# m4drat/wtf

Hardware: AMD Instinct MI355X
Metric: execs/sec + emulated instr/s per node (tlv_server, HEVD) at 1/2/4/8 GPUs (higher is better)
Workload: dtype u64

## Files before the change

wtf_amd/csrc/engine_fast.h:

```cpp
#pragma once
#include "engine_ops.h"

namespace wtfgpu_dev {

enum : u32 {
  FO_GENERIC = 0,
  FO_NOP,
  FO_MOV,
  FO_ALU,
  FO_LEA,
  FO_INCDEC,
  FO_JCC,
  FO_JMP,
  FO_CALL,
  FO_RET,
  FO_MOVX,
  FO_SHIFT,
  FO_CMOV,
  FO_SETCC,
  FO_BT,
  FO_UNARY,
  FO_VLD,
  FO_VST,
  FO_VMOV,
  FO_VZU,
};
enum : u32 {
  FF_AREG = 1,
  FF_BREG = 2,
  FF_EA = 4,
  FF_PUSH = 8,
  FF_POP = 16,
  FF_MR_A = 32,
  FF_MR_B = 64,
  FF_MW = 128,
  FF_WRA = 256,
  FF_FLAGS = 512,
};

constexpr u32 NOREG = 16;
constexpr u32 FR_HB = 32;

struct FOp {
  u32 w0;
  u32 fl;
  u32 w2;
  u32 pad;
  u64 disp, imm;
};

__device__ __forceinline__ u32 fo_op(const FOp &f) { return f.w0 & 0xff; }
__device__ __forceinline__ u32 fo_sub(const FOp &f) { return (f.w0 >> 8) & 0xf; }
__device__ __forceinline__ u32 fo_sz(const FOp &f) { return (f.w0 >> 12) & 0xf; }
__device__ __forceinline__ u32 fo_szb(const FOp &f) { return (f.w0 >> 16) & 0xf; }
__device__ __forceinline__ u32 fo_len(const FOp &f) { return (f.w0 >> 20) & 0x3f; }
__device__ __forceinline__ u32 fo_scale(const FOp &f) { return (f.w0 >> 26) & 3; }
__device__ __forceinline__ u32 fo_riprel(const FOp &f) { return (f.w0 >> 28) & 1; }
__device__ __forceinline__ u32 fo_seg(const FOp &f) { return (f.w0 >> 29) & 3; }
__device__ __forceinline__ u32 fo_ra(const FOp &f) { return f.w2 & 0xff; }
__device__ __forceinline__ u32 fo_rb(const FOp &f) { return (f.w2 >> 8) & 0xff; }
__device__ __forceinline__ u32 fo_base(const FOp &f) { return (f.w2 >> 16) & 0xff; }
__device__ __forceinline__ u32 fo_index(const FOp &f) { return (f.w2 >> 24) & 0xff; }

__device__ __forceinline__ u32 loc_regno(const UOp &u, u32 loc) {
  switch (loc) {
    case L_GREG: return u.reg;
    case L_RM: return u.is_mem ? NOREG : u.rm;
    case L_RAX: return 0;
    case L_OPREG: return u.opreg;
    default: return NOREG;
  }
}

__device__ __forceinline__ void digest_sse(const UOp &u, u32 &op, u32 &sub, u32 &ra, u32 &rb, u32 &sz) {
  const u32 x = u.opreg, c = u.sub, pp = u.bsz;
  const bool vex = x & 1;
  if (vex_map(x) != 1 || (x & 0x30000)) return;
  const u32 vvvv = vex ? (x >> 4) & 15 : 0;
  sz = vex && ((x >> 1) & 1) ? 4 : 2;
  sub = vex ? 2 : 0;
  if (vex && c == 0x77) {
    if (sz == 2) op = FO_VZU;
    return;
  }
  const bool load = ((c == 0x6f) && (pp == 1 || pp == 2)) || ((c == 0x10 || c == 0x28) && pp <= 1);
  const bool store = ((c == 0x7f) && (pp == 1 || pp == 2)) || ((c == 0x11 || c == 0x29) && pp <= 1);
  const bool aligned = c == 0x28 || c == 0x29 || (pp == 1 && (c == 0x6f || c == 0x7f));
  if ((load || store) && vvvv == 0) {
    if (aligned) sub |= 1;
    if (!u.is_mem) op = FO_VMOV, ra = load ? u.reg : u.rm, rb = load ? u.rm : u.reg;
    else op = load ? FO_VLD : FO_VST, ra = u.reg;
    return;
  }
  if (((c == 0xef && pp == 1) || (c == 0x57 && pp <= 1)) && !u.is_mem && (vex ? vvvv : u.reg) == u.rm)
    op = FO_VMOV, sub |= 4, ra = u.reg, rb = u.rm;
}

__device__ __forceinline__ void digest(const UOp &u, FOp &f) {
  u32 op = FO_GENERIC, fl = 0, sub = u.sub;
  const u32 ra = loc_regno(u, u.asrc), rb = loc_regno(u, u.bsrc);
  const bool amem = u.asrc == L_RM && u.is_mem;
  const bool bmem = u.bsrc == L_RM && u.is_mem;
  const bool areg = ra != NOREG, breg = rb != NOREG, bimm = u.bsrc == L_IMM;
  const bool hba = !u.rex && u.asz == 1 && areg && ra >= 4 && ra < 8;
  const bool hbb = !u.rex && u.bsz == 1 && breg && rb >= 4 && rb < 8;
  const bool hb = (hba || hbb) &&
                  !(u.op == O_ALU || u.op == O_TEST || u.op == O_MOV || u.op == O_MOVZX || u.op == O_MOVSX ||
                    u.op == O_INCDEC || u.op == O_NOT || u.op == O_NEG || u.op == O_SETCC || u.op == O_SHIFT);
  u64 imm = u.imm;
  u32 ra_ = ra, rb_ = rb, sz_ = u.asz;
  if (u.op == O_SSE && u.supported && !u.seg && !u.p67) {
    digest_sse(u, op, sub, ra_, rb_, sz_);
  } else if (u.supported && !u.p67 && !u.rep && !hb) {
    switch (u.op) {
      case O_NOP: op = FO_NOP; break;
      case O_MOV:
// ... 313 lines not shown
```

wtf_amd/csrc/engine_run.h:

```cpp
#pragma once
#include <hip/hip_runtime.h>

#include "engine_fast.h"

using namespace wtfgpu_dev;

namespace {

__device__ __forceinline__ u64 wave_sum(u64 v) {
#pragma unroll
  for (int off = 32; off > 0; off >>= 1) v += __shfl_xor(v, off, 64);
  return v;
}
__device__ __forceinline__ u64 readlane64(u64 v, int l) {
  const u32 lo = __builtin_amdgcn_readlane((u32)v, l);
  const u32 hi = __builtin_amdgcn_readlane((u32)(v >> 32), l);
  return ((u64)hi << 32) | lo;
}
__device__ __forceinline__ u64 m_eq32(u32 a, u32 b) { return __builtin_amdgcn_uicmp(a, b, 32); }
__device__ __forceinline__ u64 m_ne32(u32 a, u32 b) { return __builtin_amdgcn_uicmp(a, b, 33); }
__device__ __forceinline__ u64 m_eq64(u64 a, u64 b) { return __builtin_amdgcn_uicmpl(a, b, 32); }
__device__ __forceinline__ u64 m_ne64(u64 a, u64 b) { return __builtin_amdgcn_uicmpl(a, b, 33); }
__device__ __forceinline__ u64 m_lt64(u64 a, u64 b) { return __builtin_amdgcn_uicmpl(a, b, 36); }
__device__ __forceinline__ u64 m_ge64(u64 a, u64 b) { return __builtin_amdgcn_uicmpl(a, b, 35); }
// ... 143 lines not shown

__device__ __noinline__ u32 cover_edge(const Dev &P, u64 e, bool mine, u32 lane, u32 gen, u32 cnt) {
  if (!mine) return cnt;
  if (P.extra_keys && set_has(P.extra_keys, P.extra_mask, e)) return cnt;
  return log_value(P, e, true, lane, gen, cnt);
}

__device__ __forceinline__ u32 log_value(const Dev &P, u64 rip, bool mine, u32 lane, u32 gen, u32 cnt) {
  if (!mine) return cnt;
  const u32 H = P.H;
  const u64 base = (u64)lane * H;
  u32 h = (u32)mix64(rip) & (H - 1);
  for (u32 probe = 0; probe < H; probe++) {
    const u64 idx = base + h;
    if (P.cov_gen[idx] != gen) {
      if (cnt >= H - H / 4) {
        P.cov_overflow[lane] = 1;
        return cnt;
      }
      P.cov_rip[idx] = rip;
      P.cov_gen[idx] = gen;
      return cnt + 1;
    }
    if (P.cov_rip[idx] == rip) return cnt;
    h = (h + 1) & (H - 1);
  }
  return cnt;
}

__device__ __forceinline__ void fetch_bytes(u64 pageptr, u32 off, u32 n, u64 &lo, u64 &hi) {
  const u64 a = (pageptr + off) & ~7ull;
  const u32 sh = (u32)((pageptr + off) & 7);
  const u64 pend = pageptr + WTFGPU_PAGE_SIZE;
  const u64 w0 = rfl64(*(const u64 *)a);
  const u64 w1 = (a + 8 < pend) ? rfl64(*(const u64 *)(a + 8)) : 0;
  const u64 w2 = (a + 16 < pend) ? rfl64(*(const u64 *)(a + 16)) : 0;
  if (sh == 0) {
    lo = w0;
    hi = w1;
  } else {
    lo = (w0 >> (8 * sh)) | (w1 << (64 - 8 * sh));
    hi = (w1 >> (8 * sh)) | (w2 << (64 - 8 * sh));
  }
  if (n < 16) {
    if (n <= 8) {
      hi = 0;
      lo = n == 8 ? lo : (lo & ((1ull << (8 * n)) - 1));
    } else {
      hi &= (1ull << (8 * (n - 8))) - 1;
    }
  }
}

constexpr u32 UC_N = 312;
constexpr u32 UC_U = 4;
constexpr u32 UC_BP = 1, UC_COVERED = 2, UC_CROSS = 4, UC_BADLEN = 8, UC_UNSUP = 16;
struct UCHead {
  u64 key;
  u64 logged;
  u32 flags, pad;
  FOp f;
};
struct UCEntry {
  union {
    UCHead h;
    struct {
      u64 key;
      u64 logged;
      u32 flags, pad;
      FOp f;
    };
  };
  u64 rip;
};
struct UCUop {
  u64 key;
  UOp u;
};
struct GPayload {
  u32 flags, pad;
  FOp f;
  UOp u;
};
constexpr u32 GP_HEAD = (sizeof(u32) * 2 + sizeof(FOp)) / 4;
static_assert(sizeof(UOp) % 4 == 0 && sizeof(FOp) % 4 == 0, "copied as dwords");
static_assert(sizeof(UCEntry) == 64, "LDS entry size");
constexpr u32 UC_QUEUES = 2;
constexpr u64 UC_IMAGE_BYTES = (u64)UC_N * sizeof(UCEntry);

constexpr u32 UC_WAYS = 2;
static_assert(UC_N % UC_WAYS == 0, "whole sets");
__device__ __forceinline__ bool cacheable_key(u64 lptr, u64 pool_lo, u64 pool_span) {
  return !m_ge64(lptr - pool_lo, pool_span);
}
__device__ __forceinline__ u32 uc_slot(u64 key) {
  const u32 h = ((u32)key ^ (u32)(key >> 17)) * 0x9E3779B1u;
  return __umulhi(h, UC_N / UC_WAYS) * UC_WAYS;
}
__device__ __forceinline__ u32 uu_slot(u64 key) { return (u32)((key ^ (key >> 12) * 0x9E3779B1u) & (UC_U - 1)); }

template <typename T>
__device__ __forceinline__ void lds_uniform_read(const T *src, T &dst) {
  const u32 *s = (const u32 *)src;
  u32 *d = (u32 *)&dst;
#pragma unroll
  for (u32 i = 0; i < sizeof(T) / 4; i++) d[i] = rfl32(s[i]);
}

__device__ __forceinline__ void uc_head_read(const UCEntry *e, UCHead &h) {
  h.key = rfl64(e->key);
  h.flags = rfl32(e->flags);
  h.f.w0 = rfl32(e->f.w0);
  h.f.fl = rfl32(e->f.fl);
  h.f.w2 = rfl32(e->f.w2);
  h.f.disp = rfl64(e->f.disp);
  h.f.imm = rfl64(e->f.imm);
}

__device__ __forceinline__ bool bp_lookup(const Dev &P, u64 rip) {
  u32 s;
  return P.bp_keys && hash_find(P.bp_keys, P.bp_mask, rip, s);
}

__device__ __forceinline__ bool lane_phys_write(const Dev &P, Lane &L, u64 gpa, const u8 *src, u64 len) {
  while (len) {
    const u64 off = gpa & 0xfff;
    u64 n = 4096 - off;
    if (n > len) n = len;
    bool priv;
    const u8 *pg = phys_page(P, L.lane, L.ovn, L.bloom, gpa >> 12, priv);
    u8 *dst = (u8 *)pg;
    if (!priv) {
      dst = ov_alloc(P, L.lane, L.ovn);
      if (!dst) return false;
      cow_copy(P, L.lane, L.ovn, gpa >> 12, pg, dst);
      L.ovn++;
      L.bloom |= bloom_bit(gpa >> 12);
    }
    for (u64 i = 0; i < n; i++) dst[off + i] = src[i];
    src += n;
    gpa += n;
    len -= n;
  }
  return true;
}

__device__ __forceinline__ bool lane_phys_write64(const Dev &P, Lane &L, u64 gpa, u64 v) {
  bool priv;
  const u8 *pg = phys_page(P, L.lane, L.ovn, L.bloom, gpa >> 12, priv);
  u8 *dst = (u8 *)pg;
  if (!priv) {
    dst = ov_alloc(P, L.lane, L.ovn);
    if (!dst) return false;
    cow_copy(P, L.lane, L.ovn, gpa >> 12, pg, dst);
    L.ovn++;
    L.bloom |= bloom_bit(gpa >> 12);
  }
  *(u64 *)(dst + (gpa & 0xfff)) = v;
  return true;
}

__device__ __forceinline__ bool has_error_code(u32 vec) {
  return vec == 8 || (vec >= 10 && vec <= 14) || vec == 17 || vec == 21 || vec == 29 || vec == 30;
}
__device__ __forceinline__ bool sup_xlate(const Dev &P, Lane &L, u64 va, int acc, u64 &gpa) {
  u64 td, gpfn;
  if (!walk(P, L, va, acc, td, gpfn)) return false;
  gpa = (gpfn << 12) | (va & 0xfff);
  return true;
}
// ... 53 lines not shown
    L.flush = 0;
    ok = true;
  } while (0);
  if (!ok) {
    L.cpl = cpl0;
    L.status = st0;
    L.exvec = vec;
    L.exerr = err;
    L.exaddr = cr2;
    L.nodeliver = 1;
  }
  return ok;
}

constexpr u32 GUC_WORDS = 48;
constexpr u32 GUC_PAYLOAD = sizeof(GPayload) / 4;
static_assert(GUC_PAYLOAD <= 3 * 14, "global uop cache entry: 3 lines of 14 payload dwords");
__device__ __forceinline__ u32 guc_slot(const Dev &P, u64 key) {
  return (u32)(mix64(key) & P.guc_mask);
}
__device__ __forceinline__ u32 guc_payload_index(u32 lid) {
  return (lid < GUC_WORDS && (lid & 15) < 14) ? (lid >> 4) * 14 + (lid & 15) : ~0u;
}

__device__ __forceinline__ u32 covered_flag(const Dev &P, u64 rip, u32 off) {
  if (P.code_keys) {
    u32 s;
    if (hash_find(P.code_keys, P.code_mask, rip >> 12, s)) {
      const u32 cs = rfl32(P.code_slot[s]);
      if (rfl32(P.cov_map[(u64)cs * WTFGPU_PAGE_SIZE + off])) return UC_COVERED;
    }
  }
  return 0;
}

__device__ __forceinline__ u32 covered_flag_lane(const Dev &P, u64 rip, u32 off) {
  if (!P.code_keys) return 0;
  u32 h = (u32)mix64(rip >> 12) & P.code_mask;
  for (u32 i = 0; i <= P.code_mask; i++) {
    const u64 k = P.code_keys[h];
    if (k == (rip >> 12)) return P.cov_map[(u64)P.code_slot[h] * WTFGPU_PAGE_SIZE + off] ? UC_COVERED : 0;
    if (k == EMPTY_KEY) return 0;
    h = (h + 1) & P.code_mask;
  }
  return 0;
}

__device__ __forceinline__ FOp generic_fop(const UOp &d) {
  FOp f{};
  f.w0 = (d.len & 0x3f) << 20;
  return f;
}

__device__ __forceinline__ bool uc_fill_shared(const Dev &P, UCEntry *e, UCUop *us, u64 key, u32 off, u64 rip,
                                               u32 lid) {
  if (!P.guc) return false;
  const u32 pj = guc_payload_index(lid);
  u32 *head = e ? (u32 *)&e->flags : nullptr, *uop = us ? (u32 *)&us->u : nullptr;
  u32 *gw = P.guc + (u64)guc_slot(P, key) * GUC_WORDS;
  const u32 w = lid < GUC_WORDS ? gw[lid] : 0;
  const bool tag = lid < GUC_WORDS && (lid & 15) >= 14;
  const bool bad = tag && w != ((lid & 1) ? (u32)(key >> 32) : (u32)key);
  if (__ballot(bad) != 0) return false;
  if (pj < GP_HEAD) {
    if (head) head[pj] = w;
  } else if (pj < GUC_PAYLOAD) {
    if (uop) uop[pj - GP_HEAD] = w;
  }
  const u32 sflags = __builtin_amdgcn_readlane(w, 0);
  u32 flags = sflags;
  if (e && !(sflags & UC_COVERED)) {
    flags |= covered_flag(P, rip, off);
    if ((flags & UC_COVERED) && lid == 0) gw[0] = flags;
  }
  __builtin_amdgcn_wave_barrier();
  if (lid == 0) {
    if (us) us->key = key;
    if (e) {
      e->logged = 0;
      e->flags = flags;
      e->rip = rip;
      e->key = key;
    }
  }
  return true;
}

__device__ __noinline__ void uc_fill(const Dev &P, UCEntry *e, UCUop *us, u64 key, u64 lptr, u32 off, u64 rip,
                                     u32 lid, bool shared_checked = false) {
  const u32 pj = guc_payload_index(lid);
  u32 *uop = (u32 *)&us->u;
  if (!shared_checked && uc_fill_shared(P, e, us, key, off, rip, lid)) return;
  u32 *gw = P.guc ? P.guc + (u64)guc_slot(P, key) * GUC_WORDS : nullptr;
  IBytes ib;
  ib.avail = 4096 - off < 16 ? 4096 - off : 16;
  fetch_bytes(lptr, off, ib.avail, ib.lo, ib.hi);
  UOp d;
  const int dr = decode(ib, d);
  u32 flags = dr == 1 ? UC_CROSS : dr == 2 ? UC_BADLEN : 0;
  FOp f;
  if (dr == 0) {
    digest(d, f);
    if (P.edges && edge_op(d.op, d.bsrc)) f = generic_fop(d);
    if (P.trace || g_tn.buf) f = generic_fop(d);
    if (!d.supported) flags |= UC_UNSUP;
    if (bp_lookup(P, rip)) flags |= UC_BP;
  } else {
    f = FOp{};
  }
  const u32 dyn = (dr == 0 && e) ? covered_flag(P, rip, off) : 0;
  if (lid == 0) {
    us->u = d;
    us->key = key;
  }
  __builtin_amdgcn_wave_barrier();
  __builtin_amdgcn_fence(__ATOMIC_RELEASE, "wavefront");
  if (gw) {
    u32 v = 0;
    if (pj < GP_HEAD) v = pj == 0 ? (flags | dyn) : pj == 1 ? 0u : ((const u32 *)&f)[pj - 2];
    else if (pj < GUC_PAYLOAD) v = uop[pj - GP_HEAD];
    else if (lid < GUC_WORDS && (lid & 15) >= 14) v = (lid & 1) ? (u32)(key >> 32) : (u32)key;
    if (lid < GUC_WORDS) gw[lid] = v;
  }
  if (lid == 0 && e) {
    e->logged = 0;
    e->f = f;
    e->flags = flags | dyn;
    e->rip = rip;
    e->key = key;
  }
}

__device__ __forceinline__ const UOp *uc_uop(const Dev &P, UCUop *uu, u64 key, u64 lptr, u32 off, u64 rip, u32 lid) {
  UCUop *us = &uu[uu_slot(key)];
  if (rfl64(us->key) != key) uc_fill(P, nullptr, us, key, lptr, off, rip, lid);
  return &us->u;
}

__device__ __noinline__ void code_xlate(const Dev &P, Lane &L, u64 rip) {
  u64 td;
  const u64 vpn = rip >> 12;
  if (!tlb_get(L, vpn, td) || !perm_ok(L, td, ACC_X)) {
    if (service_miss(P, L, rip & ~0xfffull, ACC_X)) tlb_get(L, vpn, td);
    else td = 0;
    if (td && !perm_ok(L, td, ACC_X)) td = 0;
    if (!td && L.status == WTFGPU_EXIT_FAULT) L.exaddr = rip;
  }
  if (td) {
    L.cvpn = vpn;
    L.cptr = (td & ~0xfffull) | (L.efer & EFER_M32);
  }
}

__device__ __noinline__ bool miss_service(const Dev &P, Lane &L, int attempt) {
  if (attempt >= 16 || !service_miss(P, L, L.miss_va, (int)L.miss_acc)) {
    if (attempt >= 16) set_fault(L, WTFGPU_VEC_GP, 0xffff, L.miss_va);
    return false;
  }
  return true;
}

__device__ __noinline__ int exec_generic(const Dev &P, Lane &L, const UOp *ul, u64 &next) {
  UOp d;
  lds_uniform_read(ul, d);
  return exec(P, L, d, L.rip + d.len, next);
}

__device__ __noinline__ int exec_retry(const Dev &P, Lane &L, const UOp *ul, u64 &next) {
  int x;
  tn_insn_begin(L.lane);
  for (int attempt = 0;; attempt++) {
    L.miss = 0;
    L.pend = 0;
    tn_rollback(L.lane);
    x = exec_generic(P, L, ul, next);
    if (!L.miss || L.status != WTFGPU_RUNNING) break;
    if (!miss_service(P, L, attempt)) break;
  }
  return x;
}

__device__ __forceinline__ void retire(const Dev &P, Lane &L, int x, u32 len, u64 next, u32 opbytes) {
  if (L.flush) {
    tlb_flush(L);
    L.flush = 0;
  }
  if ((x == X_OK || x == X_CR3) && L.status == WTFGPU_RUNNING) {
    L.rip = next;
// ... 331 lines not shown
    Lane &T = C_.l;                               \
    u32 *const tlo_ = C_.r, *const thi_ = C_.r + 16; \
    _Pragma("unroll") for (int i_ = 0; i_ < 16; i_++) { \
      tlo_[i_] = glo[i_];                         \
      thi_[i_] = ghi[i_];                         \
    }                                             \
    T = L;                                        \
    T.glo = tlo_;                                 \
    T.ghi = thi_;                                 \
    call;                                         \
    L = T;                                        \
    L.glo = glo;                                  \
    L.ghi = ghi;                                  \
    _Pragma("unroll") for (int i_ = 0; i_ < 16; i_++) { \
      glo[i_] = tlo_[i_];                         \
      ghi[i_] = thi_[i_];                         \
    }                                             \
  } while (0)

#ifdef WTFGPU_STAMPS
#define STAMP(k)                                   \
  do {                                             \
    const u64 t_ = __builtin_amdgcn_s_memtime();   \
    stamp_[k] += t_ - tprev_;                      \
    tprev_ = t_;                                   \
  } while (0)
#define WHY(k) why_ = (k)
#define OPHIST(op) ophist_[((op) & 63) | (why_ & 3) << 6 | ((op) & 64 ? 256 : 0)]++
constexpr u32 STAT_N = 536;
#else
constexpr u32 STAT_N = 16;
#define OPHIST(op) \
  do {             \
  } while (0)
#define STAMP(k) \
  do {           \
  } while (0)
#define WHY(k) \
  do {         \
  } while (0)
#endif

#define RECONVERGE() __builtin_amdgcn_wave_barrier()

constexpr u32 FILL_PREFETCH = 8;
__global__ __launch_bounds__(256, 2) void k_run(Dev P, u32 first, u32 count, u64 max_steps) {
  if (P.perm && rfl64(P.stat[3]) == 0) return;
  const u32 lid = threadIdx.x & 63;
  const u32 hw = rfl32(blockIdx.x * 4 + (threadIdx.x >> 6));
  const u32 tid = hw * P.lpw + lid;
  const bool inrange = lid < P.lpw && tid < count && first + tid < P.nlanes;
  const u32 lane = inrange ? (P.perm ? P.perm[first + tid] : first + tid) : 0;
  const bool valid = inrange && P.status[lane] == WTFGPU_RUNNING;
  __shared__ UCEntry sUC[4][UC_N];
  __shared__ UCUop sUU[4][UC_U];
  UCEntry *uc = sUC[threadIdx.x >> 6];
  UCUop *uu = sUU[threadIdx.x >> 6];
  const bool wave_live = __ballot(valid) != 0;
  const UCEntry *img = (P.warm && wave_live) ? (const UCEntry *)P.warm + (u64)(hw % P.warm_n) * UC_N : nullptr;
  if (img) {
    for (u32 i = lid; i < UC_N; i += 64) {
      UCEntry t = img[i];
      t.logged = 0;
      if (P.cov_rip && t.key != EMPTY_KEY && !(t.flags & (UC_COVERED | UC_CROSS | UC_BADLEN)))
        t.flags |= covered_flag_lane(P, t.rip, (u32)(t.rip & 0xfff));
      uc[i] = t;
    }
  } else {
    for (u32 i = lid; i < UC_N; i += 64) uc[i].key = EMPTY_KEY;
  }
  if (lid < UC_U) uu[lid].key = EMPTY_KEY;
  u32 glo[16], ghi[16];
  Lane L;
  L.glo = glo;
  L.ghi = ghi;
  if (valid) {
    load_lane(P, lane, L);
  } else {
    L.status = WTFGPU_EXIT_IDLE;
    L.lane = 0;
    L.rip = 0;
    L.icount = 0;
    L.cvpn = EMPTY_KEY;
  }
  const u64 icount0 = L.icount;
  bool skip = valid && (P.lflags[lane] & 1);
  if (valid && g_tn.buf && (g_tn.pos[lane] == 0 || (P.lflags[lane] & 2))) WITH_LANE_COPY(tn_regs(P, T));
  const bool cov_on = rfl32(P.cov_rip != nullptr ? 1u : 0u) != 0;
  u64 pool_lo = (u64)(uintptr_t)P.pool, pool_span = (P.npool + 1) * WTFGPU_PAGE_SIZE;
  u64 limit_v = P.limit ? P.limit : ~0ull;
  u32 max32 = max_steps > 0xffffffffull ? 0xffffffffu : (u32)max_steps;
  asm volatile("" : "+v"(pool_lo), "+v"(pool_span), "+v"(limit_v), "+v"(max32));
  const FastMem fm = fast_mem(P);
  u32 steps = 0;
#ifdef WTFGPU_STAMPS
  u64 stamp_[8] = {0, 0, 0, 0, 0, 0, 0, 0};
  u64 tprev_ = __builtin_amdgcn_s_memtime();
  u64 whyc_[4] = {0, 0, 0, 0};
  u32 why_ = 3;
  u32 ophist_[512] = {};
  u64 bpcyc_[8] = {};
#endif

  for (;;) {
    u64 grip = 0;
    bool have = false;
    for (;;) {
      if (m_ge32(steps, max32)) break;
      const u64 am = m_eq32(L.status, WTFGPU_RUNNING);
      if (am == 0) break;
      grip = readlane64(L.rip, __ffsll((long long)am) - 1);
      u64 gm = am & m_eq64(L.rip, grip);
      if (gm != am) {
        for (u64 lo = am & m_lt64(L.rip, grip); lo; lo = am & m_lt64(L.rip, grip))
          grip = readlane64(L.rip, __ffsll((long long)lo) - 1);
        gm = am & m_eq64(L.rip, grip);
      }
      have = true;
      WHY(1);
      if (const u64 cxm = gm & m_ne64(L.cvpn, grip >> 12)) {
        if (in_mask(cxm)) {
          u64 td, gp;
          bool ok = tlb_get(L, grip >> 12, td) && perm_ok(L, td, ACC_X);
          if (!ok && fast_walk(P, L, grip & ~0xfffull, ACC_X, td, gp) && perm_ok(L, td, ACC_X)) {
            tlb_put(L, grip >> 12, td);
            ok = true;
          }
          if (ok) {
            L.cvpn = grip >> 12;
            L.cptr = (td & ~0xfffull) | (L.efer & EFER_M32);
          }
        }
        if (gm & m_ne64(L.cvpn, grip >> 12)) break;
      }
      WHY(3);
      const u64 lptr = readlane64(L.cptr, __ffsll((long long)gm) - 1);
      if (m_ge64(lptr - pool_lo, pool_span)) break;
      const u64 ingm = gm & m_eq64(L.cptr, lptr);
      const bool ing = in_mask(ingm);
      const u64 key = lptr | (grip & 0xfff);
      UCEntry *e = &uc[uc_slot(key)];
      UCHead h;
      uc_head_read(e, h);
      if (h.key != key) uc_head_read(++e, h);
      WHY(2);
      if (h.key != key) break;
      WHY(3);
      const u32 flags = h.flags;
      if (flags & (UC_CROSS | UC_BADLEN | UC_UNSUP)) break;
      if ((flags & UC_BP) && (ingm & ~__ballot(skip))) break;
      if (cov_on && !(flags & UC_COVERED) && (ingm & ~rfl64(e->logged))) break;
      const FOp &f = h.f;
      if (fo_op(f) == FO_GENERIC) break;
      if (!(f.fl & (FF_PUSH | FF_POP | FF_MR_A | FF_MR_B | FF_MW)) && fo_op(f) < FO_VLD) {
        steps++;
        have = false;
        if (ing) {
          skip = false;
          const u32 len = fo_len(f);
          FOp fr = f;
          asm volatile("" : "+s"(fr.w0), "+s"(fr.fl), "+s"(fr.w2), "+s"(fr.disp), "+s"(fr.imm));
          u64 next;
          fast_exec<true>(fm, L, fr, grip + len, next);
          L.rip = next;
          L.icount++;
          L.nbytes += len;
          if (L.icount > limit_v) L.status = WTFGPU_EXIT_TIMEOUT;
        }
        RECONVERGE();
        continue;
      }
      steps++;
      have = false;
      STAMP(6);
      const u32 len = fo_len(f);
      u64 next = 0;
      u64 wantm = ingm;
      if (ing) skip = false;
      for (u32 round = 0;; round++) {
        if (in_mask(wantm)) {
          L.miss = 0;
          L.pend = 0;
          FOp fr = f;
          asm volatile("" : "+s"(fr.w0), "+s"(fr.fl), "+s"(fr.w2), "+s"(fr.disp), "+s"(fr.imm));
          fast_exec(fm, L, fr, grip + len, next);
        }
        RECONVERGE();
        wantm = round >= 3 ? 0 : wantm & m_eq32(L.miss, 2);
        if (wantm == 0) break;
        u64 csrc = 0, cdst = 0, cgpfn = 0, ctd = 0;
        bool want = in_mask(wantm);
        if (want && !fast_fill_prep(P, L, csrc, cdst, cgpfn, ctd)) {
          want = false;
          fast_fault(P, L);
        }
        for (u64 cm = __ballot(want && cdst); cm; cm &= cm - 1) {
          const int l = __ffsll((long long)cm) - 1;
          const uint4 *s4 = (const uint4 *)(uintptr_t)readlane64(csrc, l) + lid * 4;
          uint4 *d4 = (uint4 *)(uintptr_t)readlane64(cdst, l) + lid * 4;
          const uint4 a = s4[0], b = s4[1], c = s4[2], d = s4[3];
          d4[0] = a;
          d4[1] = b;
          d4[2] = c;
          d4[3] = d;
        }
        __builtin_amdgcn_fence(__ATOMIC_ACQ_REL, "workgroup");
        if (want && cdst) fast_fill_finish(P, L, cdst, cgpfn, ctd);
        wantm = __ballot(want);
      }
      const u64 missm = ingm & m_ne32(L.miss, 0);
      if (in_mask(ingm & ~missm)) {
        L.rip = next;
        L.icount++;
        L.nbytes += len + L.pend;
        if (L.icount > limit_v) L.status = WTFGPU_EXIT_TIMEOUT;
      }
      RECONVERGE();
      STAMP(7);
      if (missm & m_eq32(L.status, WTFGPU_RUNNING)) {
        WHY(0);
        steps--;
        have = true;
        break;
      }
      if (missm) break;
    }
    STAMP(0);
    if (__ballot(L.status == WTFGPU_EXIT_FAULT && !L.nodeliver)) {
      if (L.status == WTFGPU_EXIT_FAULT && !L.nodeliver) {
        bool dv;
        WITH_LANE_COPY(dv = deliver_fault(P, T));
        if (dv && g_tn.buf) WITH_LANE_COPY(tn_regs(P, T));
      }
      RECONVERGE();
      continue;
    }
    if (!have) break;

    steps++;
#ifdef WTFGPU_STAMPS
    whyc_[why_ & 3]++;
#endif
    const bool active = L.status == WTFGPU_RUNNING;
    bool cand = active && L.rip == grip;
    if (cand && (grip >> 12) != L.cvpn) WITH_LANE_COPY(code_xlate(P, T, grip));
    cand = cand && (grip >> 12) == L.cvpn;
    const u64 cm = __ballot(cand);
    if (cm == 0) continue;
    const int leader = __ffsll((long long)cm) - 1;
    const u64 lptr = readlane64(L.cptr, leader);
    bool ing = cand && L.cptr == lptr;

    const u32 off = (u32)(grip & 0xfff);
    const u64 key = lptr | off;
    UCEntry *e = &uc[uc_slot(key)];
    if (rfl64(e->key) != key) {
      if (rfl64(e[1].key) == key) e += 1;
      else if (cacheable_key(lptr, pool_lo, pool_span)) {
        if (lid < 16) ((u32 *)&e[1])[lid] = ((const u32 *)e)[lid];
        __builtin_amdgcn_wave_barrier();
      }
    }
    const bool cacheable = !m_ge64(lptr - pool_lo, pool_span);
    if (cacheable && rfl64(e->key) != key) {
      if (!uc_fill_shared(P, e, &uu[uu_slot(key)], key, off, grip, lid))
        uc_fill(P, e, &uu[uu_slot(key)], key, lptr, off, grip, lid, true);
      const UCEntry *pe = e;
      u64 prip = grip;
      for (u32 k = 0; k < FILL_PREFETCH; k++) {
        const u32 pf = rfl32(pe->flags), pw0 = rfl32(pe->f.w0), plen = (pw0 >> 20) & 0x3f;
        if ((pf & (UC_CROSS | UC_BADLEN)) || !plen) break;
        const u64 nxt = prip + plen;
        if ((nxt >> 12) != (grip >> 12) || (nxt & 0xfff) > 4096 - 16) break;
        const u32 poff = (u32)(nxt & 0xfff);
        const u64 pkey = lptr | poff;
        UCEntry *ps = &uc[uc_slot(pkey)];
        if (rfl64(ps->key) == pkey || rfl64(ps[1].key) == pkey) break;
        if (!uc_fill_shared(P, ps + 1, nullptr, pkey, poff, nxt, lid)) break;
        pe = ps + 1;
        prip = nxt;
      }
      const u32 ff = rfl32(e->flags);
      if (!(ff & (UC_BP | UC_CROSS | UC_BADLEN | UC_UNSUP)) && (!cov_on || (ff & UC_COVERED)) &&
          (rfl32(e->f.w0) & 0xff) != FO_GENERIC) {
        steps--;
        STAMP(2);
        continue;
      }
    }
    STAMP(2);
    const u32 flags = cacheable ? rfl32(e->flags) : UC_CROSS;
    if (flags & (UC_CROSS | UC_BADLEN)) {
      if (flags & UC_BADLEN) {
        if (ing) set_fault(L, WTFGPU_VEC_GP, 0, 0);
      } else if (L.status != WTFGPU_EXIT_IDLE) {
        bool sk = skip;
        WITH_LANE_COPY(slow_step(P, T, grip, lptr, ing, sk));
        skip = sk;
      }
      RECONVERGE();
      STAMP(5);
      continue;
    }
    const u32 len = (rfl32(e->f.w0) >> 20) & 0x3f;
    const u64 gmask = __ballot(ing);

    if (P.trace && ing && !skip) trace_rip(P, L.lane, grip);
    bool logged_now = false;
    if (cov_on && !(flags & UC_COVERED)) {
      const u64 logged = rfl64(e->logged);
      if (gmask & ~logged) {
        L.ccnt = cover(P, grip, ing && !((logged >> lid) & 1), L.lane, L.cgen, L.ccnt);
        if (lid == 0) e->logged = logged | gmask;
        logged_now = true;
      }
    }
    STAMP(3);
    if (logged_now && !(flags & (UC_BP | UC_UNSUP)) && (rfl32(e->f.w0) & 0xff) != FO_GENERIC) {
      steps--;
      continue;
    }
    u32 act_kind = ~0u;
    const wtfgpu_bp_action_t *act = nullptr;
    if ((flags & UC_BP) && P.act_keys && !g_tn.buf) {
      u32 slot;
      if (hash_find(P.act_keys, P.act_mask, grip, slot)) {
        act = &P.act[slot];
        act_kind = rfl32(act->kind);
      }
    }
#ifdef WTFGPU_STAMPS
    if (__ballot(ing && (flags & UC_BP) && !skip)) OPHIST(56 + (act_kind < 7 ? act_kind : 7));
#endif
    if (act_kind == WTFGPU_BPACT_SET_GPRS && ing && !skip) {
#pragma unroll
      for (u32 i = 0; i < 16; i++) RS(L, i, act->gprs[i]);
      L.rip = act->gprs[16];
      skip = L.rip == grip;
      ing = false;
    }
    if (act_kind == WTFGPU_BPACT_STOP_OK && ing && !skip) {
      L.status = WTFGPU_EXIT_STOP_OK;
      skip = true;
      ing = false;
    }
    if (act_kind == WTFGPU_BPACT_FEED && P.feed_pos) {
      bool want = false;
      if (ing && !skip) {
        const u64 pos = P.feed_pos[L.lane];
        const u64 end = P.feed_end[L.lane];
        if (pos != ~0ull && pos + 4 <= end) {
          const u8 *src = P.feed_data + pos;
          const u32 n = (u32)src[0] | ((u32)src[1] << 8) | ((u32)src[2] << 16) | ((u32)src[3] << 24);
          const u64 win = act->value;
          if (n && n < win && pos + 4 + n <= end) {
            const u64 va = R(L, (u32)act->gprs[0] & 15) + win - n;
            u64 td;
            if (!(tlb_get(L, va >> 12, td) && (td & T_PRIV))) {
              L.miss_va = va;
              L.miss_acc = ACC_W;
              want = true;
            }
          }
        }
      }
      u64 csrc = 0, cdst = 0, cgpfn = 0, ctd = 0;
      if (want) {
        const u32 cpl0 = L.cpl;
        const u64 cr00 = L.cr0;
        L.cpl = 0;
        L.cr0 &= ~(1ull << 16);
// ... 12 lines not shown
        d4[2] = c;
        d4[3] = d;
      }
      __builtin_amdgcn_fence(__ATOMIC_ACQ_REL, "workgroup");
      if (want && cdst) fast_fill_finish(P, L, cdst, cgpfn, ctd);
      RECONVERGE();
    }
    if (ing) {
      if ((flags & UC_BP) && !skip) {
        bool applied = false;
#ifdef WTFGPU_STAMPS
        const u64 tb_ = __builtin_amdgcn_s_memtime();
#endif
        if (P.act_keys) WITH_LANE_COPY(applied = bp_apply(P, T, grip, act));
#ifdef WTFGPU_STAMPS
        bpcyc_[act_kind < 7 ? act_kind : 7] += __builtin_amdgcn_s_memtime() - tb_;
#endif
        if (!applied) L.status = WTFGPU_EXIT_BREAKPOINT;
        skip = applied && L.rip == grip;
        if (applied && !skip && g_tn.buf) WITH_LANE_COPY(tn_regs(P, T));
        ing = false;
      } else {
        skip = false;
      }
    }
    STAMP(4);
    const UOp *u = nullptr;
    if (__ballot(ing)) u = uc_uop(P, uu, key, lptr, off, grip, lid);
    if (__ballot(ing) && !(flags & UC_UNSUP)) OPHIST(rfl32(u->op) + (flags & UC_COVERED ? 64 : 0));
    if (ing && (flags & UC_UNSUP)) {
      const u32 ob = u->opbytes, n = len;
      L.status = WTFGPU_EXIT_UNIMPLEMENTED;
      L.exop = n >= 4 ? ob : (ob & ((1u << (8 * n)) - 1));
      ing = false;
    }
    if (ing) {
      u64 next = 0;
      int x;
      WITH_LANE_COPY(x = exec_retry(P, T, u, next));
      u32 opbytes = 0;
      if (x == X_UNIMPL) opbytes = u->opbytes;
      retire(P, L, x, len, next, opbytes);
      if (g_tn.buf && (x == X_OK || x == X_CR3)) WITH_LANE_COPY(tn_regs(P, T));
      if (P.edges && P.cov_rip && x == X_OK && edge_op(rfl32(u->op), rfl32(u->bsrc))) {
        const u32 c0 = L.ccnt;
        L.ccnt = cover_edge(P, edge_key(grip, next), true, L.lane, L.cgen, L.ccnt);
        count_edge(P, L.lane, L.ccnt != c0);
      }
    }
    RECONVERGE();
    STAMP(1);
  }

  if (P.warm && wave_live && hw < P.warm_n) {
    __builtin_amdgcn_wave_barrier();
    __builtin_amdgcn_fence(__ATOMIC_ACQUIRE, "wavefront");
    UCEntry *out = (UCEntry *)P.warm + (u64)hw * UC_N;
    for (u32 i = lid; i < UC_N; i += 64) out[i] = uc[i];
  }
  if (valid && g_tn.buf && L.status != WTFGPU_RUNNING && L.status != WTFGPU_EXIT_BREAKPOINT &&
      g_tn.pos[lane] > g_tn.ipos[lane])
    WITH_LANE_COPY(tn_regs(P, T));
  if (valid) {
    store_lane(P, L);
    store_tlb(P, L);
    if (L.status == WTFGPU_EXIT_FAULT || L.status == WTFGPU_EXIT_UNIMPLEMENTED) {
      ExitInfo ei;
      ei.vector = L.exvec;
      ei.error = L.exerr;
      ei.opcode = L.exop;
      ei.cpl = L.cpl;
      ei.addr = L.exaddr;
      P.exinfo[lane] = ei;
    }
    P.lflags[lane] = skip ? 1u : 0u;
  }
  const u64 retired = wave_sum(valid ? L.icount - icount0 : 0);
  const u64 running = wave_sum((valid && L.status == WTFGPU_RUNNING) ? 1 : 0);
  if (lid == 0) {
    atomicAdd((unsigned long long *)&P.stat[0], (unsigned long long)steps);
    atomicAdd((unsigned long long *)&P.stat[1], (unsigned long long)retired);
    if (running) atomicAdd((unsigned long long *)&P.stat[2], (unsigned long long)running);
#ifdef WTFGPU_STAMPS
    for (int k = 0; k < 8; k++) atomicAdd((unsigned long long *)&P.stat[4 + k], (unsigned long long)stamp_[k]);
    for (int k = 0; k < 4; k++) atomicAdd((unsigned long long *)&P.stat[12 + k], (unsigned long long)whyc_[k]);
    for (int k = 0; k < 512; k++)
      if (ophist_[k]) atomicAdd((unsigned long long *)&P.stat[16 + k], (unsigned long long)ophist_[k]);
    for (int k = 0; k < 8; k++) atomicAdd((unsigned long long *)&P.stat[528 + k], (unsigned long long)bpcyc_[k]);
#endif
  }
}

}
```

Measured before the change: 14.98 million.

## Compact LDS uop-cache heads to 32 bytes and grow cache capacity

Replaces the 64-byte per-wave LDS cache entry with a 32-byte aligned head. The head packs the decoded-op flags and cache flags into one word and narrows disp to 32 bits; entries whose displacement does not fit fall back to the generic path. The per-entry logged mask moves to a separate LDS array, and the rip moves out of LDS into the global warm image. The freed LDS space raises the entry count from 312 to 500, and head reads become two 16-byte loads. The aim is fewer uop-cache misses and cheaper lookups, at the cost of extra pack/unpack work, a narrower disp, and more LDS per block, which may limit occupancy.

After: 15.24 million (median of 2 runs). No clear change (+1.8%).

```diff
diff --git a/wtf_amd/csrc/engine_fast.h b/wtf_amd/csrc/engine_fast.h
--- a/wtf_amd/csrc/engine_fast.h
+++ b/wtf_amd/csrc/engine_fast.h
@@ -62,6 +62,38 @@
 __device__ __forceinline__ u32 fo_base(const FOp &f) { return (f.w2 >> 16) & 0xff; }
 __device__ __forceinline__ u32 fo_index(const FOp &f) { return (f.w2 >> 24) & 0xff; }
 
+constexpr u32 UC_BP = 1, UC_COVERED = 2, UC_CROSS = 4, UC_BADLEN = 8, UC_UNSUP = 16;
+constexpr u32 UCH_FLAGS_SHIFT = 16;
+struct alignas(32) UCHead {
+  u64 key;
+  u32 w0;
+  u32 ff;
+  u32 w2;
+  i32 disp;
+  u64 imm;
+};
+static_assert(sizeof(UCHead) == 32 && alignof(UCHead) == 32, "LDS head: two aligned 16-byte reads");
+static_assert(FF_FLAGS < (1u << UCH_FLAGS_SHIFT) && UC_UNSUP < (1u << (32 - UCH_FLAGS_SHIFT)), "one word holds both");
+
+__host__ __device__ __forceinline__ void uc_head_pack(u64 key, u32 flags, const FOp &f, UCHead &h) {
+  const bool fits = (u64)(i64)(i32)(u32)f.disp == f.disp;
+  h.key = key;
+  h.w0 = fits ? f.w0 : (f.w0 & (0x3fu << 20));
+  h.ff = (fits ? f.fl : 0u) | flags << UCH_FLAGS_SHIFT;
+  h.w2 = fits ? f.w2 : 0u;
+  h.disp = fits ? (i32)(u32)f.disp : 0;
+  h.imm = fits ? f.imm : 0ull;
+}
+__host__ __device__ __forceinline__ void uc_head_unpack(const UCHead &h, u32 &flags, FOp &f) {
+  flags = h.ff >> UCH_FLAGS_SHIFT;
+  f.w0 = h.w0;
+  f.fl = h.ff & ((1u << UCH_FLAGS_SHIFT) - 1);
+  f.w2 = h.w2;
+  f.pad = 0;
+  f.disp = (u64)(i64)h.disp;
+  f.imm = h.imm;
+}
+
 __device__ __forceinline__ u32 loc_regno(const UOp &u, u32 loc) {
   switch (loc) {
     case L_GREG: return u.reg;
diff --git a/wtf_amd/csrc/engine_run.h b/wtf_amd/csrc/engine_run.h
--- a/wtf_amd/csrc/engine_run.h
+++ b/wtf_amd/csrc/engine_run.h
@@ -219,30 +219,21 @@
   }
 }
 
-constexpr u32 UC_N = 312;
+constexpr u32 UC_N = 500;
 constexpr u32 UC_U = 4;
-constexpr u32 UC_BP = 1, UC_COVERED = 2, UC_CROSS = 4, UC_BADLEN = 8, UC_UNSUP = 16;
-struct UCHead {
-  u64 key;
-  u64 logged;
-  u32 flags, pad;
-  FOp f;
-};
-struct UCEntry {
-  union {
-    UCHead h;
-    struct {
-      u64 key;
-      u64 logged;
-      u32 flags, pad;
-      FOp f;
-    };
-  };
-  u64 rip;
-};
 struct UCUop {
   u64 key;
   UOp u;
+};
+struct UCWave {
+  UCHead h[UC_N];
+  u64 logged[UC_N];
+  UCUop uu[UC_U];
+};
+static_assert(sizeof(UCWave) * 4 <= 80 * 1024, "two blocks of four waves per CU");
+struct UCache {
+  UCWave *w;
+  u64 *rip;
 };
 struct GPayload {
   u32 flags, pad;
@@ -251,9 +242,15 @@
 };
 constexpr u32 GP_HEAD = (sizeof(u32) * 2 + sizeof(FOp)) / 4;
 static_assert(sizeof(UOp) % 4 == 0 && sizeof(FOp) % 4 == 0, "copied as dwords");
-static_assert(sizeof(UCEntry) == 64, "LDS entry size");
 constexpr u32 UC_QUEUES = 2;
-constexpr u64 UC_IMAGE_BYTES = (u64)UC_N * sizeof(UCEntry);
+constexpr u64 UC_IMAGE_BYTES = (u64)UC_N * (sizeof(UCHead) + sizeof(u64));
+
+__device__ __forceinline__ u8 *uc_image_out(const Dev &P, u32 hw, bool keeps) {
+  return keeps ? P.warm + (u64)hw * UC_IMAGE_BYTES : nullptr;
+}
+__device__ __forceinline__ u64 *uc_image_rips(const u8 *img) {
+  return img ? (u64 *)(uintptr_t)(img + (u64)UC_N * sizeof(UCHead)) : nullptr;
+}
 
 constexpr u32 UC_WAYS = 2;
 static_assert(UC_N % UC_WAYS == 0, "whole sets");
@@ -274,15 +271,22 @@
   for (u32 i = 0; i < sizeof(T) / 4; i++) d[i] = rfl32(s[i]);
 }
 
-__device__ __forceinline__ void uc_head_read(const UCEntry *e, UCHead &h) {
-  h.key = rfl64(e->key);
-  h.flags = rfl32(e->flags);
-  h.f.w0 = rfl32(e->f.w0);
-  h.f.fl = rfl32(e->f.fl);
-  h.f.w2 = rfl32(e->f.w2);
-  h.f.disp = rfl64(e->f.disp);
-  h.f.imm = rfl64(e->f.imm);
-}
+__device__ __forceinline__ void uc_head_read(const UCHead *e, UCHead &h) {
+  const uint4 *p = (const uint4 *)e;
+  const uint4 a = p[0], b = p[1];
+  h.key = (u64)rfl32(a.x) | (u64)rfl32(a.y) << 32;
+  h.w0 = rfl32(a.z);
+  h.ff = rfl32(a.w);
+  h.w2 = rfl32(b.x);
+  h.disp = (i32)rfl32(b.y);
+  h.imm = (u64)rfl32(b.z) | (u64)rfl32(b.w) << 32;
+}
+__device__ __forceinline__ void uc_head_write(UCHead *e, const UCHead &h) {
+  uint4 *p = (uint4 *)e;
+  p[0] = make_uint4((u32)h.key, (u32)(h.key >> 32), h.w0, h.ff);
+  p[1] = make_uint4(h.w2, (u32)h.disp, (u32)h.imm, (u32)(h.imm >> 32));
+}
+__device__ __forceinline__ u32 uc_flags(const UCHead *e) { return rfl32(e->ff) >> UCH_FLAGS_SHIFT; }
 
 __device__ __forceinline__ bool bp_lookup(const Dev &P, u64 rip) {
   u32 s;
@@ -442,45 +446,58 @@
   return f;
 }
 
-__device__ __forceinline__ bool uc_fill_shared(const Dev &P, UCEntry *e, UCUop *us, u64 key, u32 off, u64 rip,
-                                               u32 lid) {
+__device__ __forceinline__ void uc_entry_write(const UCache &uc, u32 i, u64 key, u32 flags, const FOp &f, u64 rip) {
+  UCHead h;
+  uc_head_pack(key, flags, f, h);
+  uc.w->logged[i] = 0;
+  if (uc.rip) uc.rip[i] = rip;
+  uc_head_write(&uc.w->h[i], h);
+}
+
+__device__ __forceinline__ bool uc_fill_shared(const Dev &P, const UCache uc, u32 ei, UCUop *us, u64 key, u32 off,
+                                               u64 rip, u32 lid) {
   if (!P.guc) return false;
   const u32 pj = guc_payload_index(lid);
-  u32 *head = e ? (u32 *)&e->flags : nullptr, *uop = us ? (u32 *)&us->u : nullptr;
+  u32 *uop = us ? (u32 *)&us->u : nullptr;
   u32 *gw = P.guc + (u64)guc_slot(P, key) * GUC_WORDS;
   const u32 w = lid < GUC_WORDS ? gw[lid] : 0;
   const bool tag = lid < GUC_WORDS && (lid & 15) >= 14;
   const bool bad = tag && w != ((lid & 1) ? (u32)(key >> 32) : (u32)key);
   if (__ballot(bad) != 0) return false;
-  if (pj < GP_HEAD) {
-    if (head) head[pj] = w;
-  } else if (pj < GUC_PAYLOAD) {
+  if (pj >= GP_HEAD && pj < GUC_PAYLOAD) {
     if (uop) uop[pj - GP_HEAD] = w;
   }
   const u32 sflags = __builtin_amdgcn_readlane(w, 0);
   u32 flags = sflags;
-  if (e && !(sflags & UC_COVERED)) {
+  if (uc.w && !(sflags & UC_COVERED)) {
     flags |= covered_flag(P, rip, off);
     if ((flags & UC_COVERED) && lid == 0) gw[0] = flags;
+  }
+  static_assert(GP_HEAD == 10 && sizeof(FOp) == 32, "the FOp's dwords in the shared payload");
+  FOp f;
+  if (uc.w) {
+    const u32 d6 = __builtin_amdgcn_readlane(w, 6), d7 = __builtin_amdgcn_readlane(w, 7);
+    const u32 d8 = __builtin_amdgcn_readlane(w, 8), d9 = __builtin_amdgcn_readlane(w, 9);
+    f.w0 = __builtin_amdgcn_readlane(w, 2);
+    f.fl = __builtin_amdgcn_readlane(w, 3);
+    f.w2 = __builtin_amdgcn_readlane(w, 4);
+    f.pad = 0;
+    f.disp = (u64)d6 | (u64)d7 << 32;
+    f.imm = (u64)d8 | (u64)d9 << 32;
   }
   __builtin_amdgcn_wave_barrier();
   if (lid == 0) {
     if (us) us->key = key;
-    if (e) {
-      e->logged = 0;
-      e->flags = flags;
-      e->rip = rip;
-      e->key = key;
-    }
+    if (uc.w) uc_entry_write(uc, ei, key, flags, f, rip);
   }
   return true;
 }
 
-__device__ __noinline__ void uc_fill(const Dev &P, UCEntry *e, UCUop *us, u64 key, u64 lptr, u32 off, u64 rip,
-                                     u32 lid, bool shared_checked = false) {
+__device__ __noinline__ void uc_fill(const Dev &P, const UCache uc, u32 ei, UCUop *us, u64 key, u64 lptr, u32 off,
+                                     u64 rip, u32 lid, bool shared_checked = false) {
   const u32 pj = guc_payload_index(lid);
   u32 *uop = (u32 *)&us->u;
-  if (!shared_checked && uc_fill_shared(P, e, us, key, off, rip, lid)) return;
+  if (!shared_checked && uc_fill_shared(P, uc, ei, us, key, off, rip, lid)) return;
   u32 *gw = P.guc ? P.guc + (u64)guc_slot(P, key) * GUC_WORDS : nullptr;
   IBytes ib;
   ib.avail = 4096 - off < 16 ? 4096 - off : 16;
@@ -498,7 +515,7 @@
   } else {
     f = FOp{};
   }
-  const u32 dyn = (dr == 0 && e) ? covered_flag(P, rip, off) : 0;
+  const u32 dyn = (dr == 0 && uc.w) ? covered_flag(P, rip, off) : 0;
   if (lid == 0) {
     us->u = d;
     us->key = key;
@@ -512,18 +529,12 @@
     else if (lid < GUC_WORDS && (lid & 15) >= 14) v = (lid & 1) ? (u32)(key >> 32) : (u32)key;
     if (lid < GUC_WORDS) gw[lid] = v;
   }
-  if (lid == 0 && e) {
-    e->logged = 0;
-    e->f = f;
-    e->flags = flags | dyn;
-    e->rip = rip;
-    e->key = key;
-  }
+  if (lid == 0 && uc.w) uc_entry_write(uc, ei, key, flags | dyn, f, rip);
 }
 
 __device__ __forceinline__ const UOp *uc_uop(const Dev &P, UCUop *uu, u64 key, u64 lptr, u32 off, u64 rip, u32 lid) {
   UCUop *us = &uu[uu_slot(key)];
-  if (rfl64(us->key) != key) uc_fill(P, nullptr, us, key, lptr, off, rip, lid);
+  if (rfl64(us->key) != key) uc_fill(P, UCache{nullptr, nullptr}, 0, us, key, lptr, off, rip, lid);
   return &us->u;
 }
 
@@ -961,19 +972,33 @@
   const bool inrange = lid < P.lpw && tid < count && first + tid < P.nlanes;
   const u32 lane = inrange ? (P.perm ? P.perm[first + tid] : first + tid) : 0;
   const bool valid = inrange && P.status[lane] == WTFGPU_RUNNING;
-  __shared__ UCEntry sUC[4][UC_N];
-  __shared__ UCUop sUU[4][UC_U];
-  UCEntry *uc = sUC[threadIdx.x >> 6];
-  UCUop *uu = sUU[threadIdx.x >> 6];
+  __shared__ UCWave sUC[4];
+  UCWave *ucv = &sUC[threadIdx.x >> 6];
+  UCHead *uc = ucv->h;
+  u64 *ulog = ucv->logged;
+  UCUop *uu = ucv->uu;
   const bool wave_live = __ballot(valid) != 0;
-  const UCEntry *img = (P.warm && wave_live) ? (const UCEntry *)P.warm + (u64)(hw % P.warm_n) * UC_N : nullptr;
+  const u8 *img = (P.warm && wave_live) ? P.warm + (u64)(hw % P.warm_n) * UC_IMAGE_BYTES : nullptr;
+  const bool keeps_img = P.warm && wave_live && hw < P.warm_n;
   if (img) {
+    const UCHead *ih = (const UCHead *)img;
+    const u64 *ir = uc_image_rips(img);
     for (u32 i = lid; i < UC_N; i += 64) {
-      UCEntry t = img[i];
-      t.logged = 0;
-      if (P.cov_rip && t.key != EMPTY_KEY && !(t.flags & (UC_COVERED | UC_CROSS | UC_BADLEN)))
-        t.flags |= covered_flag_lane(P, t.rip, (u32)(t.rip & 0xfff));
-      uc[i] = t;
+      const uint4 a = ((const uint4 *)&ih[i])[0], b = ((const uint4 *)&ih[i])[1];
+      UCHead t;
+      t.key = (u64)a.x | (u64)a.y << 32;
+      t.w0 = a.z, t.ff = a.w, t.w2 = b.x, t.disp = (i32)b.y;
+      t.imm = (u64)b.z | (u64)b.w << 32;
+      u32 tf;
+      FOp f;
+      uc_head_unpack(t, tf, f);
+      if (P.cov_rip && t.key != EMPTY_KEY && !(tf & (UC_COVERED | UC_CROSS | UC_BADLEN))) {
+        const u64 rip = ir[i];
+        tf |= covered_flag_lane(P, rip, (u32)(rip & 0xfff));
+        uc_head_pack(t.key, tf, f, t);
+      }
+      uc_head_write(&uc[i], t);
+      ulog[i] = 0;
     }
   } else {
     for (u32 i = lid; i < UC_N; i += 64) uc[i].key = EMPTY_KEY;
@@ -992,7 +1017,6 @@
     L.icount = 0;
     L.cvpn = EMPTY_KEY;
   }
-  const u64 icount0 = L.icount;
   bool skip = valid && (P.lflags[lane] & 1);
   if (valid && g_tn.buf && (g_tn.pos[lane] == 0 || (P.lflags[lane] & 2))) WITH_LANE_COPY(tn_regs(P, T));
   const bool cov_on = rfl32(P.cov_rip != nullptr ? 1u : 0u) != 0;
@@ -1048,18 +1072,19 @@
       const u64 ingm = gm & m_eq64(L.cptr, lptr);
       const bool ing = in_mask(ingm);
       const u64 key = lptr | (grip & 0xfff);
-      UCEntry *e = &uc[uc_slot(key)];
+      u32 ei = uc_slot(key);
       UCHead h;
-      uc_head_read(e, h);
-      if (h.key != key) uc_head_read(++e, h);
+      uc_head_read(&uc[ei], h);
+      if (h.key != key) uc_head_read(&uc[++ei], h);
       WHY(2);
       if (h.key != key) break;
       WHY(3);
-      const u32 flags = h.flags;
+      u32 flags;
+      FOp f;
+      uc_head_unpack(h, flags, f);
       if (flags & (UC_CROSS | UC_BADLEN | UC_UNSUP)) break;
       if ((flags & UC_BP) && (ingm & ~__ballot(skip))) break;
-      if (cov_on && !(flags & UC_COVERED) && (ingm & ~rfl64(e->logged))) break;
-      const FOp &f = h.f;
+      if (cov_on && !(flags & UC_COVERED) && (ingm & ~rfl64(ulog[ei]))) break;
       if (fo_op(f) == FO_GENERIC) break;
       if (!(f.fl & (FF_PUSH | FF_POP | FF_MR_A | FF_MR_B | FF_MW)) && fo_op(f) < FO_VLD) {
         steps++;
@@ -1162,43 +1187,50 @@
 
     const u32 off = (u32)(grip & 0xfff);
     const u64 key = lptr | off;
-    UCEntry *e = &uc[uc_slot(key)];
+    u32 ei = uc_slot(key);
+    const UCHead *e = &uc[ei];
+    const UCache ucw{ucv, uc_image_rips(uc_image_out(P, hw, keeps_img))};
     if (rfl64(e->key) != key) {
-      if (rfl64(e[1].key) == key) e += 1;
-      else if (cacheable_key(lptr, pool_lo, pool_span)) {
-        if (lid < 16) ((u32 *)&e[1])[lid] = ((const u32 *)e)[lid];
+      if (rfl64(e[1].key) == key) {
+        e = &uc[++ei];
+      } else if (cacheable_key(lptr, pool_lo, pool_span)) {
+        if (lid < 8) ((u32 *)&uc[ei + 1])[lid] = ((const u32 *)&uc[ei])[lid];
+        if (lid == 0) {
+          ulog[ei + 1] = ulog[ei];
+          if (ucw.rip) ucw.rip[ei + 1] = ucw.rip[ei];
+        }
         __builtin_amdgcn_wave_barrier();
       }
     }
     const bool cacheable = !m_ge64(lptr - pool_lo, pool_span);
     if (cacheable && rfl64(e->key) != key) {
-      if (!uc_fill_shared(P, e, &uu[uu_slot(key)], key, off, grip, lid))
-        uc_fill(P, e, &uu[uu_slot(key)], key, lptr, off, grip, lid, true);
-      const UCEntry *pe = e;
+      if (!uc_fill_shared(P, ucw, ei, &uu[uu_slot(key)], key, off, grip, lid))
+        uc_fill(P, ucw, ei, &uu[uu_slot(key)], key, lptr, off, grip, lid, true);
+      const UCHead *pe = e;
       u64 prip = grip;
       for (u32 k = 0; k < FILL_PREFETCH; k++) {
-        const u32 pf = rfl32(pe->flags), pw0 = rfl32(pe->f.w0), plen = (pw0 >> 20) & 0x3f;
+        const u32 pf = uc_flags(pe), pw0 = rfl32(pe->w0), plen = (pw0 >> 20) & 0x3f;
         if ((pf & (UC_CROSS | UC_BADLEN)) || !plen) break;
         const u64 nxt = prip + plen;
         if ((nxt >> 12) != (grip >> 12) || (nxt & 0xfff) > 4096 - 16) break;
         const u32 poff = (u32)(nxt & 0xfff);
         const u64 pkey = lptr | poff;
-        UCEntry *ps = &uc[uc_slot(pkey)];
-        if (rfl64(ps->key) == pkey || rfl64(ps[1].key) == pkey) break;
-        if (!uc_fill_shared(P, ps + 1, nullptr, pkey, poff, nxt, lid)) break;
-        pe = ps + 1;
+        const u32 pi = uc_slot(pkey);
+        if (rfl64(uc[pi].key) == pkey || rfl64(uc[pi + 1].key) == pkey) break;
+        if (!uc_fill_shared(P, ucw, pi + 1, nullptr, pkey, poff, nxt, lid)) break;
+        pe = &uc[pi + 1];
         prip = nxt;
       }
-      const u32 ff = rfl32(e->flags);
+      const u32 ff = uc_flags(e);
       if (!(ff & (UC_BP | UC_CROSS | UC_BADLEN | UC_UNSUP)) && (!cov_on || (ff & UC_COVERED)) &&
-          (rfl32(e->f.w0) & 0xff) != FO_GENERIC) {
+          (rfl32(e->w0) & 0xff) != FO_GENERIC) {
         steps--;
         STAMP(2);
         continue;
       }
     }
     STAMP(2);
-    const u32 flags = cacheable ? rfl32(e->flags) : UC_CROSS;
+    const u32 flags = cacheable ? uc_flags(e) : UC_CROSS;
     if (flags & (UC_CROSS | UC_BADLEN)) {
       if (flags & UC_BADLEN) {
         if (ing) set_fault(L, WTFGPU_VEC_GP, 0, 0);
@@ -1211,21 +1243,21 @@
       STAMP(5);
       continue;
     }
-    const u32 len = (rfl32(e->f.w0) >> 20) & 0x3f;
+    const u32 len = (rfl32(e->w0) >> 20) & 0x3f;
     const u64 gmask = __ballot(ing);
 
     if (P.trace && ing && !skip) trace_rip(P, L.lane, grip);
     bool logged_now = false;
     if (cov_on && !(flags & UC_COVERED)) {
-      const u64 logged = rfl64(e->logged);
+      const u64 logged = rfl64(ulog[ei]);
       if (gmask & ~logged) {
         L.ccnt = cover(P, grip, ing && !((logged >> lid) & 1), L.lane, L.cgen, L.ccnt);
-        if (lid == 0) e->logged = logged | gmask;
+        if (lid == 0) ulog[ei] = logged | gmask;
         logged_now = true;
       }
     }
     STAMP(3);
-    if (logged_now && !(flags & (UC_BP | UC_UNSUP)) && (rfl32(e->f.w0) & 0xff) != FO_GENERIC) {
+    if (logged_now && !(flags & (UC_BP | UC_UNSUP)) && (rfl32(e->w0) & 0xff) != FO_GENERIC) {
       steps--;
       continue;
     }
@@ -1344,15 +1376,16 @@
     STAMP(1);
   }
 
-  if (P.warm && wave_live && hw < P.warm_n) {
+  if (u8 *img_out = uc_image_out(P, hw, keeps_img)) {
     __builtin_amdgcn_wave_barrier();
     __builtin_amdgcn_fence(__ATOMIC_ACQUIRE, "wavefront");
-    UCEntry *out = (UCEntry *)P.warm + (u64)hw * UC_N;
-    for (u32 i = lid; i < UC_N; i += 64) out[i] = uc[i];
+    uint4 *out = (uint4 *)img_out;
+    for (u32 i = lid; i < UC_N * 2; i += 64) out[i] = ((const uint4 *)uc)[i];
   }
   if (valid && g_tn.buf && L.status != WTFGPU_RUNNING && L.status != WTFGPU_EXIT_BREAKPOINT &&
       g_tn.pos[lane] > g_tn.ipos[lane])
     WITH_LANE_COPY(tn_regs(P, T));
+  const u64 icount0 = valid ? P.icount[lane] : 0;
   if (valid) {
     store_lane(P, L);
     store_tlb(P, L);
```
